# SmartBFT-Go/consensus

Measured on AMD Instinct MI355X. Metric: ECDSA P-256 verifies/sec at batch=1M, higher is better.
Workload: dtype u32

## Files before the change

### consensus_amd/csrc/ed25519_group_kernels.hip

```cpp
#include <hip/hip_runtime.h>

#include <cstdlib>

#include "ed25519_group.h"
#include "ed25519_keyed.h"
#include "ed25519_kernels.h"
#include "group_kernels_common.h"
#include "p256_kernels.h"

namespace sbv {

#ifndef SBV_ED_QPHASE_WAVES
#define SBV_ED_QPHASE_WAVES 3
#endif
#ifndef SBV_ED_GROUP_WAVES
#define SBV_ED_GROUP_WAVES 2
#endif

#ifndef SBV_ED_CHAIN_PRIO
#define SBV_ED_CHAIN_PRIO 0
#endif
static __device__ __forceinline__ void ed_chain_prio() {
#if SBV_ED_CHAIN_PRIO > 0
    __builtin_amdgcn_s_setprio(SBV_ED_CHAIN_PRIO);
#endif
}

__global__ __launch_bounds__(256) void k_ed_group_insert(const uint8_t* __restrict__ tuples, size_t n, GroupState g) {
    const size_t i = (size_t)blockIdx.x * 256 + threadIdx.x;
    (void)i;
    group_insert_block<128, 64, 8>(tuples, n, g);
}

__global__ __launch_bounds__(256) void k_ed_group_split(size_t n, GroupState g) {
    const size_t i = (size_t)blockIdx.x * 256 + threadIdx.x;
    const bool active = i < n;
    u32 s = SBV_GROUP_NONE;
    if (active) s = g.slot_of[g.rep[i]];
    group_split_emit(i, s, active && s == SBV_GROUP_NONE, active && s != SBV_GROUP_NONE, false, g);
}

__global__ __launch_bounds__(64) void k_ed_keytab_bases(const uint8_t* __restrict__ tuples, GroupState g, u32* __restrict__ jbases,
                                                        uint8_t* __restrict__ valid, const u32* __restrict__ tslot, const uint8_t* __restrict__ cold,
                                                        int j_first, int j_last) {
    const u32 lane = blockIdx.x * 64 + threadIdx.x;
    const u32 k = lane >> 2;
    if (k >= group_count(g) || !cold[k]) return;
    edchain_quad_dev q;
    q.r = (int)(lane & 3u);
    edchain_run(q, tuples, k, g, jbases, valid + tslot[k], j_first, j_last);
}

__global__ __launch_bounds__(64) void k_ed_keytab_window(GroupState g, const u32* __restrict__ jbases, u32* __restrict__ tmp,
                                                         aniels* __restrict__ ktab, const u32* __restrict__ tslot, const uint8_t* __restrict__ cold,
                                                         int j_first, int j_count, int parts) {
    const u32 lane = blockIdx.x * 64 + threadIdx.x;
    const u32 part = lane % (u32)parts;
    const u32 kw = lane / (u32)parts;
    const u32 key = kw / (u32)j_count, j = (u32)j_first + kw % (u32)j_count;
    if (key >= group_count(g) || !cold[key]) return;
    const size_t w = (size_t)key * SBV_ED_KEY_WINDOWS + j;
    ed_keytab_window_lane(jbases + w * SBV_ED_JBASE_DWORDS, (int)part, parts,
                          tmp + w * (size_t)(SBV_ED_KEY_PER_WINDOW * SBV_ED_WINDOW_TMP_WORDS) + (size_t)part * (SBV_ED_KEY_PER_WINDOW / parts) * SBV_ED_WINDOW_TMP_WORDS,
// ... 125 lines not shown
                                                                  uint8_t* __restrict__ acc, int j0, int j1, int last) {
    const u32 L = blockIdx.x * SBV_VERIFY_BLOCK + threadIdx.x;
    if (L >= g.counters[1]) return;
    const u32 t = g.grp_idx[L];
    const u32 grp = g.slots[t];
    const bool v = ed_qphase_lane(tuples, t, grp < group_count(g) ? tslot[grp] : SBV_GROUP_NONE, table_slots, ktab, kvalid, gacc, cap, okb, j0, j1, last != 0);
    if (last) acc[t] = v ? SBV_ED_PENDING : 0;
}

__global__ __launch_bounds__(256) void k_ed_finish(const uint8_t* __restrict__ tuples, size_t n, u32* __restrict__ gacc, size_t cap,
                                                   uint8_t* __restrict__ acc, int tuple_major) {
    const size_t i0 = ((size_t)blockIdx.x * 256 + threadIdx.x) * SBV_ED_FINISH_T;
    if (i0 < n) ed_finish_lane(tuples, n, i0, gacc, cap, acc, tuple_major != 0);
}

hipError_t launch_ed25519_verify_grouped(const uint8_t* d_tuples, size_t n, const GroupBuffers& b, const EdGroupBuffers& eb,
                                         u32* d_qtab, const aniels* d_btab, const edcomb& bcomb, uint8_t* d_bitmap, hipStream_t stream,
                                         const GroupSync& y, hipEvent_t* prof, int* prof_pairs) {
    if (n == 0) return hipSuccess;
    GroupState g;
    g.ht = b.ht; g.ht_mask = b.ht_mask; g.rep = b.rep; g.cnt = b.cnt; g.slot_of = b.slot_of; g.group_rep = b.group_rep;
    g.counters = b.counters; g.grp_idx = b.grp_idx; g.ung_idx = b.ung_idx; g.slots = b.slots;
    g.max_groups = b.max_groups; g.seed = b.seed;
    g.gcount = b.gcount; g.gcursor = b.gcount ? b.gcount + b.max_groups : nullptr; g.grp_of = b.grp_of; g.ung_cand = b.ung_cand;
    const size_t sort_lds = (size_t)b.max_groups * sizeof(u32);
    g.sorted = ed25519_group_step_sorted(y, b) ? 1u : 0u;
    group_set_threshold(g, b.min_count);
    const int chunks = y.chunks < 1 ? 1 : (y.chunks > SBV_GROUP_MAX_CHUNKS ? SBV_GROUP_MAX_CHUNKS : y.chunks);
    const int parts = SBV_KEYTAB_PARTS_DEFAULT;
    hipError_t e;
#define SBV_TRY(x) do { if ((e = (x)) != hipSuccess) return e; } while (0)
    SBV_TRY(hipStreamWaitEvent(y.side_a, y.ev_fork, 0));
    SBV_TRY(hipStreamWaitEvent(y.side_a, y.ev_promoted, 0));
    SBV_TRY(hipMemsetAsync(b.ht, 0, ((size_t)b.ht_mask + 1) * sizeof(u32), y.side_a));
    SBV_TRY(hipMemsetAsync(b.cnt, 0, n * sizeof(u32), y.side_a));
    SBV_TRY(hipMemsetAsync(b.counters, 0, SBV_GROUP_COUNTERS * sizeof(u32), y.side_a));
    if (g.sorted) SBV_TRY(hipMemsetAsync(b.gcount, 0, (size_t)b.max_groups * sizeof(u32), y.side_a));
    SBV_TRY(hipMemsetAsync(b.acc, 0, n, y.side_a));
    const unsigned gn = (unsigned)((n + 255) / 256);
    const unsigned gv = (unsigned)((n + SBV_VERIFY_BLOCK - 1) / SBV_VERIFY_BLOCK);
    hipLaunchKernelGGL(k_ed_group_insert, dim3(gn), dim3(256), 0, y.side_a, d_tuples, n, g);
    hipLaunchKernelGGL((k_group_assign_t<128, 64, 8>), dim3(gn), dim3(256), 0, y.side_a, d_tuples, n, g, eb.kc);
    SBV_TRY(hipEventRecord(y.ev_assign, y.side_a));
    hipLaunchKernelGGL((k_key_cache_lookup_t<128, 64, 8>), dim3((b.max_groups + 63) / 64), dim3(64), 0, y.side_a, d_tuples, g, eb.kc, b.tslot, b.cold);
    hipLaunchKernelGGL((k_key_cache_insert_t<128, 64, 8>), dim3((b.max_groups + 63) / 64), dim3(64), 0, y.side_a, d_tuples, g, eb.kc, b.tslot);
    const u32 table_slots = eb.kc.cap + b.max_groups;
    const bool hot_on = eb.wtab && eb.kwide && eb.wide && eb.kc.enabled && g.sorted;
    const HotKeys hk = {eb.wtab, hot_on ? eb.kwide : nullptr, eb.khits, eb.hot, eb.plist, eb.kc.cap, eb.wide_cap, eb.promote_min, eb.wowner, eb.elist};
    const uint8_t* wide = hot_on ? eb.wide : nullptr;
    if (hot_on) SBV_TRY(hipEventRecord(y.ev_cache, y.side_a));
    SBV_TRY(hipStreamWaitEvent(y.side_b, y.ev_assign, 0));
    if (hot_on) SBV_TRY(hipMemsetAsync(eb.hot + 1, 0, 3 * sizeof(u32), y.side_b));
    if (g.sorted) {
        const unsigned tiles = (unsigned)((n + SBV_SORT_TILE - 1) / SBV_SORT_TILE);
        hipLaunchKernelGGL(k_group_classify, dim3(gn), dim3(256), 0, y.side_b, n, g, b.ung_cand, b.counters + 4);
        hipLaunchKernelGGL(k_group_sort_count, dim3(tiles), dim3(1024), sort_lds, y.side_b, n, g);
        hipLaunchKernelGGL(k_group_sort_scan, dim3(1), dim3(1024), 0, y.side_b, g);
        hipLaunchKernelGGL(k_group_sort_scatter, dim3(tiles), dim3(1024), sort_lds, y.side_b, n, g);
    } else {
        hipLaunchKernelGGL(k_ed_group_split, dim3(gn), dim3(256), 0, y.side_b, n, g);
    }
    if (hot_on) {
        SBV_TRY(hipStreamWaitEvent(y.side_b, y.ev_cache, 0));
        hipLaunchKernelGGL(k_ed_hot_class, dim3(64), dim3(256), 0, y.side_b, g, b.tslot, b.cold, hk, eb.wide);
    }
    SBV_TRY(hipEventRecord(y.ev_split, y.side_b));
    hipLaunchKernelGGL(k_ed_gphase, dim3(gv), dim3(SBV_VERIFY_BLOCK), 0, stream, d_tuples, n, bcomb, b.gacc, b.gacc_cap, eb.okb, (int)g.sorted);
    if (hot_on) SBV_TRY(hipEventRecord(y.ev_class, stream));
    SBV_TRY(hipStreamWaitEvent(stream, y.ev_split, 0));
    for (int c = 0; c < chunks; ++c) {
        const int j_first = SBV_ED_KEY_WINDOWS * c / chunks, j_end = SBV_ED_KEY_WINDOWS * (c + 1) / chunks;
        hipLaunchKernelGGL(k_ed_keytab_bases, dim3((b.max_groups * 4u + 63) / 64), dim3(64), 0, y.side_a, d_tuples, g, b.jbases, eb.kvalid,
                           b.tslot, b.cold, j_first, j_end - 1);
        SBV_TRY(hipEventRecord(y.ev_bases[c], y.side_a));
    }
    SBV_TRY(hipStreamWaitEvent(y.side_a, y.ev_split, 0));
    static const bool quad_env = [] { const char* e = getenv("SBV_ED_UNGROUPED_QUAD"); return e && atoi(e) != 0; }();
    static const bool keep_keys = [] { const char* e = getenv("SBV_ED_UNGROUPED_KEYS"); return !e || atoi(e) != 0; }();
// ... 130 lines not shown
```

### consensus_amd/csrc/group_kernels_common.h

```cpp
#pragma once
#include <hip/hip_runtime.h>

#include "p256_group.h"

namespace sbv {

__device__ __forceinline__ u32 group_count(const GroupState& g) {
    const u32 c = g.counters[0];
    return c < g.max_groups ? c : g.max_groups;
}

template <int STRIDE, int OFF, int WORDS>
static __device__ __forceinline__ void group_insert_block(const uint8_t* __restrict__ tuples, size_t n, const GroupState& g) {
    __shared__ u32 skey[512], scnt[512];
    const unsigned tid = threadIdx.x;
    for (unsigned t = tid; t < 512; t += blockDim.x) { skey[t] = 0xFFFFFFFFu; scnt[t] = 0; }
    __syncthreads();
    const size_t i = (size_t)blockIdx.x * blockDim.x + tid;
    u32 mine = 0xFFFFFFFFu;
    bool want = false;
    if (i < n) {
        mine = group_find_rep_t<STRIDE, OFF, WORDS>(tuples, i, g);
        want = group_sampled((u32)i, g.sample_mask);
    }
    unsigned long long todo = __ballot(want);
    const int lane = (int)(tid & 63u);
    if (todo) {
        const int first = __ffsll((long long)todo) - 1;
        const u32 r0 = (u32)__shfl((int)mine, first, 64);
        if (__popcll(__ballot(want && mine == r0)) < 2) {
            if (want) atomicAdd(&g.cnt[mine], 1u);
            todo = 0;
        }
    }
    while (todo) {
        const int leader = __ffsll((long long)todo) - 1;
        const u32 r = (u32)__shfl((int)mine, leader, 64);
        const unsigned long long same = __ballot(want && mine == r);
        if (lane == leader) {
            const u32 c = (u32)__popcll(same);
            u32 h = (r * 0x9E3779B1u) >> 23;
            for (int probes = 0; probes < 512; ++probes) {
                const u32 prev = atomicCAS(&skey[h], 0xFFFFFFFFu, r);
                if (prev == 0xFFFFFFFFu || prev == r) { atomicAdd(&scnt[h], c); break; }
                h = (h + 1u) & 511u;
            }
        }
        todo &= ~same;
    }
    __syncthreads();
    for (unsigned t = tid; t < 512; t += blockDim.x)
        if (skey[t] != 0xFFFFFFFFu) atomicAdd(&g.cnt[skey[t]], scnt[t]);
}

template <int STRIDE, int OFF, int WORDS>
static __global__ __launch_bounds__(256) void k_group_assign_t(const uint8_t* __restrict__ tuples, size_t n, GroupState g, KeyCache kc) {
    const size_t i = (size_t)blockIdx.x * 256 + threadIdx.x;
    if (i < n) group_assign_lane_t<STRIDE, OFF, WORDS>(tuples, i, g, kc);
}
static __global__ __launch_bounds__(256) void k_group_assign(const uint8_t* __restrict__ tuples, size_t n, GroupState g, KeyCache kc) {
    const size_t i = (size_t)blockIdx.x * 256 + threadIdx.x;
    if (i < n) group_assign_lane(tuples, i, g, kc);
}

template <int STRIDE, int OFF, int WORDS>
static __global__ __launch_bounds__(64) void k_key_cache_lookup_t(const uint8_t* __restrict__ tuples, GroupState g, KeyCache kc,
                                                                  u32* __restrict__ tslot, uint8_t* __restrict__ cold) {
    const u32 k = blockIdx.x * 64 + threadIdx.x;
    if (k == 0) { kc.count[1] = 0; kc.count[2] = 0; }
    if (k >= group_count(g)) return;
    key_cache_phase_lookup<STRIDE, OFF, WORDS>(tuples, g, kc, k, tslot, cold);
}
template <int STRIDE, int OFF, int WORDS>
static __global__ __launch_bounds__(64) void k_key_cache_insert_t(const uint8_t* __restrict__ tuples, GroupState g, KeyCache kc,
                                                                  u32* __restrict__ tslot) {
    const u32 k = blockIdx.x * 64 + threadIdx.x;
    if (k >= group_count(g)) return;
    key_cache_phase_insert<STRIDE, OFF, WORDS>(tuples, g, kc, k, tslot);
}

struct HotKeys { const void* wtab; u32* kwide; u32* khits; u32* hot; u32* plist; u32 cache_cap, wide_cap, promote_min; u32* wowner; u32* elist; };
static __device__ __forceinline__ u32 promote_live(const u32* hot) { const u32 c = hot[1]; return c < SBV_PROMOTE_MAX ? c : SBV_PROMOTE_MAX; }
static __global__ __launch_bounds__(256) void k_hot_decay(HotKeys hk) {
    const u32 slot = blockIdx.x * 256 + threadIdx.x;
    if (slot < hk.cache_cap) hot_decay_lane(slot, hk.khits);
}
static __global__ __launch_bounds__(256) void k_promote_select(GroupState g, const u32* __restrict__ tslot, const uint8_t* __restrict__ kvalid, HotKeys hk) {
    const u32 groups = group_count(g);
    for (u32 k = blockIdx.x * 256 + threadIdx.x; k < groups; k += gridDim.x * 256)
        group_promote_select_lane(k, tslot, kvalid, hk.cache_cap, hk.kwide, hk.khits, hk.promote_min, hk.wide_cap, hk.hot, hk.plist, hk.elist);
}
#define SBV_HOT_POOL_MAX 4096u
static __global__ __launch_bounds__(1024) void k_promote_evict(HotKeys hk) {
    __shared__ u32 taken[SBV_HOT_POOL_MAX / 32];
    __shared__ u32 sh_h[16], sh_w[16];
    __shared__ u32 entries;
    const u32 tid = threadIdx.x;
    const u32 ncand = hk.hot[3] < SBV_PROMOTE_MAX ? hk.hot[3] : SBV_PROMOTE_MAX;
    if (ncand == 0 || hk.wide_cap > SBV_HOT_POOL_MAX) return;
    for (u32 i = tid; i < SBV_HOT_POOL_MAX / 32; i += 1024) taken[i] = 0;
    if (tid == 0) entries = hk.hot[1] < SBV_PROMOTE_MAX ? hk.hot[1] : SBV_PROMOTE_MAX;
    __syncthreads();
    {
        u32 mc = 0;
        for (u32 c = tid; c < ncand; c += 1024) { const u32 h = hk.khits[hk.elist[c]]; mc = h > mc ? h : mc; }
        u32 bh, bw;
        hot_evict_scan(hk.khits, hk.wowner, taken, hk.wide_cap, hk.cache_cap, tid, 1024u, bh, bw);
        for (int off = 32; off >= 1; off >>= 1) {
            const u32 om = (u32)__shfl_xor((int)mc, off, 64), oh = (u32)__shfl_xor((int)bh, off, 64);
            mc = om > mc ? om : mc;
            bh = oh < bh ? oh : bh;
// ... 193 lines not shown
```

### consensus_amd/csrc/k256_group_kernels.hip

```cpp
#include <hip/hip_runtime.h>

#include <thread>
#include <vector>

#include "group_kernels_common.h"
#include "k256_group.h"
#include "k256_keyed.h"
#include "p256_kernels.h"

namespace sbv {

struct KGlobalTupleG {
    const u32* p;
    __device__ __forceinline__ u32 operator[](int i) const { return p[i]; }
};
#define SBV_K256_PREP_T 8
__global__ __launch_bounds__(64) void k_k256_prep_chunk(const uint8_t* __restrict__ tuples, size_t n, Scratch s, int T) {
    const size_t first = (size_t)blockIdx.x * 64 * (size_t)T + threadIdx.x;
    auto words = [&](size_t idx) { return KGlobalTupleG{reinterpret_cast<const u32*>(tuples + idx * 160)}; };
    k256_prep_chunk(words, n, s, first, (size_t)64, T);
}
__global__ __launch_bounds__(256) void k_k256_group_insert(const uint8_t* __restrict__ tuples, size_t n, GroupState g) {
    group_insert_block<160, 96, 16>(tuples, n, g);
}
// ... 123 lines not shown
}
__global__ __launch_bounds__(64) void k_k256_promote_build(const u32* __restrict__ plist, const u32* __restrict__ hot, const kapt* __restrict__ ktab, u32 cache_cap,
                                                           u32* __restrict__ tmp, kapt* __restrict__ wtab, u32 wide_cap) {
    const u32 total = promote_live(hot) * SBV_K256_WIDE_LANES;
    const u32 gid = blockIdx.x * 64 + threadIdx.x;
    u32* mine = tmp + (size_t)gid * SBV_K256_WIDE_TMP_WORDS;
    for (u32 item = gid; item < total; item += gridDim.x * 64) {
        const u32 i = item / SBV_K256_WIDE_LANES, lane = item % SBV_K256_WIDE_LANES;
        const u32 slot = plist[2 * i], w = plist[2 * i + 1];
        if (slot >= cache_cap || w >= wide_cap) continue;
        k256_widetab_lane(ktab + (size_t)slot * SBV_K256_KEYTAB_ENTRIES, lane, mine, wtab + (size_t)w * SBV_K256_WIDE_ENTRIES);
    }
}

hipError_t launch_k256_verify_grouped(const uint8_t* d_tuples, const Scratch& s_in, size_t n, const GroupBuffers& b, const KeyPool& kp, u32* d_qtab,
                                      const kapt* d_gtab, const kapt* d_gcomb, int gcomb_bits, uint8_t* d_bitmap, hipStream_t stream, const GroupSync& y, hipEvent_t* prof, int* prof_pairs) {
    if (n == 0) return hipSuccess;
    GroupState g;
    g.ht = b.ht; g.ht_mask = b.ht_mask; g.rep = b.rep; g.cnt = b.cnt; g.slot_of = b.slot_of; g.group_rep = b.group_rep;
    g.counters = b.counters; g.grp_idx = b.grp_idx; g.ung_idx = b.ung_idx; g.slots = b.slots; g.max_groups = b.max_groups; g.seed = b.seed;
    g.gcount = b.gcount; g.gcursor = b.gcount + b.max_groups; g.grp_of = b.grp_of; g.ung_cand = b.ung_cand;
    g.sorted = k256_group_step_sorted(y, b) ? 1u : 0u;
    group_set_threshold(g, b.min_count);
    Scratch s = s_in;
    s.rec = b.rec;
    const size_t sort_lds = (size_t)b.max_groups * sizeof(u32);
    kapt* ktab = reinterpret_cast<kapt*>(kp.ktab);
    uint8_t* kvalid = kp.kvalid;
    const u32 table_slots = kp.kc.cap + b.max_groups;
    hipError_t e;
#define SBV_TRY(x) do { if ((e = (x)) != hipSuccess) return e; } while (0)
    SBV_TRY(hipStreamWaitEvent(y.side_a, y.ev_fork, 0));
    SBV_TRY(hipStreamWaitEvent(y.side_a, y.ev_promoted, 0));
    SBV_TRY(hipMemsetAsync(b.ht, 0, ((size_t)b.ht_mask + 1) * sizeof(u32), y.side_a));
    SBV_TRY(hipMemsetAsync(b.cnt, 0, n * sizeof(u32), y.side_a));
    SBV_TRY(hipMemsetAsync(b.counters, 0, SBV_GROUP_COUNTERS * sizeof(u32), y.side_a));
    SBV_TRY(hipMemsetAsync(b.gcount, 0, (size_t)b.max_groups * sizeof(u32), y.side_a));
    const unsigned gn = (unsigned)((n + 255) / 256);
    const unsigned gv = (unsigned)((n + SBV_VERIFY_BLOCK - 1) / SBV_VERIFY_BLOCK);
    hipLaunchKernelGGL(k_k256_group_insert, dim3(gn), dim3(256), 0, y.side_a, d_tuples, n, g);
    hipLaunchKernelGGL(k_group_assign, dim3(gn), dim3(256), 0, y.side_a, d_tuples, n, g, kp.kc);
    SBV_TRY(hipEventRecord(y.ev_assign, y.side_a));
    hipLaunchKernelGGL((k_key_cache_lookup_t<160, 96, 16>), dim3((b.max_groups + 63) / 64), dim3(64), 0, y.side_a, d_tuples, g, kp.kc, b.tslot, b.cold);
    hipLaunchKernelGGL((k_key_cache_insert_t<160, 96, 16>), dim3((b.max_groups + 63) / 64), dim3(64), 0, y.side_a, d_tuples, g, kp.kc, b.tslot);
    const bool hot_on = kp.wtab && kp.kwide && kp.wide && kp.build_blocks && kp.kc.enabled && g.sorted;
    const HotKeys hk = {kp.wtab, hot_on ? kp.kwide : nullptr, kp.khits, kp.hot, kp.plist, kp.kc.cap, kp.wide_cap, kp.promote_min, kp.wowner, kp.elist};
    const uint8_t* wide = hot_on ? kp.wide : nullptr;
    if (hot_on) SBV_TRY(hipEventRecord(y.ev_cache, y.side_a));
    {
        const size_t per_block = (size_t)64 * SBV_K256_PREP_T;
        hipLaunchKernelGGL(k_k256_prep_chunk, dim3((unsigned)((n + per_block - 1) / per_block)), dim3(64), 0, stream, d_tuples, n, s, SBV_K256_PREP_T);
    }
    SBV_TRY(hipStreamWaitEvent(y.side_b, y.ev_assign, 0));
    if (hot_on) SBV_TRY(hipMemsetAsync(kp.hot + 1, 0, 3 * sizeof(u32), y.side_b));
    hipLaunchKernelGGL(k_group_classify, dim3(gn), dim3(256), 0, y.side_b, n, g, b.ung_cand, b.counters + 4);
    hipLaunchKernelGGL(k_k256_keycheck, dim3(gn), dim3(256), 0, y.side_b, d_tuples, g, b.acc);
    const unsigned tiles = (unsigned)((n + SBV_SORT_TILE - 1) / SBV_SORT_TILE);
    hipLaunchKernelGGL(k_group_sort_count, dim3(tiles), dim3(1024), sort_lds, y.side_b, n, g);
    hipLaunchKernelGGL(k_group_sort_scan, dim3(1), dim3(1024), 0, y.side_b, g);
    hipLaunchKernelGGL(k_group_sort_scatter, dim3(tiles), dim3(1024), sort_lds, y.side_b, n, g);
    if (hot_on) {
        SBV_TRY(hipStreamWaitEvent(y.side_b, y.ev_cache, 0));
        hipLaunchKernelGGL(k_k256_hot_class, dim3(64), dim3(256), 0, y.side_b, g, b.tslot, b.cold, hk, kp.wide);
    }
    SBV_TRY(hipEventRecord(y.ev_split, y.side_b));
    SBV_TRY(hipStreamWaitEvent(stream, y.ev_split, 0));
    hipLaunchKernelGGL(k_k256_gphase_generic, dim3(2 * gv), dim3(SBV_VERIFY_BLOCK), 0, stream, s, g, d_qtab, d_gtab, kgcomb_make(d_gcomb, gcomb_bits), b.gacc, b.acc, gv);
    if (hot_on) SBV_TRY(hipEventRecord(y.ev_class, stream));
    const int chunks = 2;
    for (int c = 0; c < chunks; ++c) {
        const int j_first = SBV_GTAB_WINDOWS * c / chunks, j_end = SBV_GTAB_WINDOWS * (c + 1) / chunks, j_count = j_end - j_first;
        hipLaunchKernelGGL(k_k256_chain, dim3((b.max_groups * 4 + 63) / 64), dim3(64), 0, y.side_a, d_tuples, g, b.jstate, b.bases, kvalid, b.tslot, b.cold, j_first, j_end - 1);
        SBV_TRY(hipEventRecord(y.ev_bases[c], y.side_a));
        hipStream_t tb = y.tstreams > 1 && y.side_t && (c & 1) ? y.side_t : y.side_b;
        SBV_TRY(hipStreamWaitEvent(tb, y.ev_bases[c], 0));
        const size_t wl = (size_t)b.max_groups * j_count * 2, fl = (size_t)b.max_groups * j_count * 7;
        hipLaunchKernelGGL(k_k256_rows, dim3((unsigned)((wl + 63) / 64)), dim3(64), 0, tb, g, b.bases, b.tmp, ktab, b.tslot, b.cold, j_first, j_count);
// ... 41 lines not shown
```

### consensus_amd/csrc/p256_group.h

```cpp
#pragma once
#include "p256_core.h"
#include "p256_comb29.h"

namespace sbv {

#if defined(__HIP_DEVICE_COMPILE__)
#define SBV_ATOMIC_CAS(p, cmp, val) atomicCAS((p), (cmp), (val))
#define SBV_ATOMIC_ADD(p, v) atomicAdd((p), (v))
#else
SBV_HD u32 host_cas(u32* p, u32 cmp, u32 val) { const u32 old = *p; if (old == cmp) *p = val; return old; }
SBV_HD u32 host_add(u32* p, u32 v) { const u32 old = *p; *p = old + v; return old; }
#define SBV_ATOMIC_CAS(p, cmp, val) host_cas((p), (cmp), (val))
#define SBV_ATOMIC_ADD(p, v) host_add((p), (v))
#endif

#define SBV_GROUP_NONE 0xFFFFFFFFu
#define SBV_GROUP_COUNTERS 12
#define SBV_GROUP_MAX_PROBES 64u

struct GroupState {
    u32* ht;
    u32 ht_mask;
    u32* rep;
    u32* cnt;
// ... 30 lines not shown
    h ^= h >> 15;
    h *= 0x85EBCA77u;
    return ((h >> 24) & sample_mask) == 0;
}

SBV_HD const u32* tuple_key_words(const uint8_t* tuples, size_t i) {
    return reinterpret_cast<const u32*>(tuples + i * 160 + 96);
}

SBV_HD bool key29_load(const uint8_t* tuples, size_t idx, fe29& x, fe29& y) {
    const u32* k = tuple_key_words(tuples, idx);
    u256 qx, qy;
    SBV_UNROLL
    for (int l = 0; l < 8; ++l) { qx.v[l] = bswap32(k[7 - l]); qy.v[l] = bswap32(k[8 + 7 - l]); }
    const fe p_ = fe_p();
    f29_from_plain(x, qx);
    f29_from_plain(y, qy);
    fe29 lhs, t, rhs;
    f29_sqr(lhs, y);
    f29_sqr(t, x);
    f29_mul(rhs, t, x);
    f29_sub(rhs, rhs, x);
    f29_sub(rhs, rhs, x);
    f29_sub(rhs, rhs, x);
    f29_add(rhs, rhs, f29_b());
    f29_sub(t, lhs, rhs);
    return lt256(qx, p_) && lt256(qy, p_) && f29_is_zero(t);
}
SBV_HD bool tuple_key_ok(const uint8_t* tuples, size_t idx) {
    fe29 x, y;
    return key29_load(tuples, idx, x, y);
}

template <int STRIDE, int OFF, int WORDS>
SBV_HD u32 group_find_rep_t(const uint8_t* tuples, size_t i, const GroupState& g) {
    const u32* k = reinterpret_cast<const u32*>(tuples + i * STRIDE + OFF);
    u32 w[WORDS];
    SBV_UNROLL
    for (int j = 0; j < WORDS; ++j) w[j] = k[j];
    u32 h = 0x9E3779B1u ^ g.seed;
    SBV_UNROLL
    for (int j = 0; j < WORDS; ++j) {
        h = (h ^ w[j]) * 0x85EBCA77u;
        h ^= h >> 15;
    }
    h = (h ^ (g.seed * 0x27D4EB2Fu)) * 0xC2B2AE3Du;
    h ^= h >> 16;
    u32 slot = h & g.ht_mask;
    u32 mine = (u32)i;
    for (u32 probes = 0; probes < SBV_GROUP_MAX_PROBES && probes <= g.ht_mask; ++probes) {
        u32 v = g.ht[slot];
        if (v == 0) v = SBV_ATOMIC_CAS(&g.ht[slot], 0u, (u32)i + 1u);
        if (v == 0) break;
        const u32* o = reinterpret_cast<const u32*>(tuples + (size_t)(v - 1) * STRIDE + OFF);
        u32 diff = 0;
        SBV_UNROLL
        for (int j = 0; j < WORDS; ++j) diff |= o[j] ^ w[j];
        if (diff == 0) { mine = v - 1; break; }
        slot = (slot + 1) & g.ht_mask;
    }
    g.rep[i] = mine;
    return mine;
}
template <int STRIDE, int OFF, int WORDS>
SBV_HD void group_insert_lane_t(const uint8_t* tuples, size_t i, const GroupState& g) {
    const u32 mine = group_find_rep_t<STRIDE, OFF, WORDS>(tuples, i, g);
    if (group_sampled((u32)i, g.sample_mask)) SBV_ATOMIC_ADD(&g.cnt[mine], 1u);
}
SBV_HD void group_insert_lane(const uint8_t* tuples, size_t i, const GroupState& g) { group_insert_lane_t<160, 96, 16>(tuples, i, g); }

SBV_HD bool group_split_lane(const uint8_t* tuples, size_t i, const GroupState& g, uint8_t* acc) {
    const u32 s = g.slot_of[g.rep[i]];
    if (s == SBV_GROUP_NONE) {
        g.slots[i] = SBV_GROUP_NONE;
        if (!tuple_key_ok(tuples, i)) {
            acc[i] = 0;
            SBV_ATOMIC_ADD(&g.counters[3], 1u);
            return false;
        }
        g.ung_idx[SBV_ATOMIC_ADD(&g.counters[2], 1u)] = (u32)i;
    } else {
        g.slots[i] = s;
        if (!g.sorted) g.grp_idx[SBV_ATOMIC_ADD(&g.counters[1], 1u)] = (u32)i;
    }
    return true;
}

// ... 43 lines not shown
struct KeyCache {
    u32* ht;
    u32 ht_mask;
    u32* keys;
    u32* count;
    u32 cap;
    u32 enabled;
    u32 seed;
};
SBV_HD u32 key_hash16(const u32 w[16], u32 seed) {
    u32 h = 0x9E3779B1u ^ seed;
    SBV_UNROLL
    for (int j = 0; j < 16; ++j) {
        h = (h ^ w[j]) * 0x85EBCA77u;
        h ^= h >> 15;
    }
    h = (h ^ (seed * 0x27D4EB2Fu)) * 0xC2B2AE3Du;
    return h ^ (h >> 16);
}
SBV_HD u32 key_cache_lookup(const KeyCache& kc, const u32 w[16]) {
    u32 p = key_hash16(w, kc.seed) & kc.ht_mask;
    for (u32 probes = 0; probes < SBV_GROUP_MAX_PROBES && probes <= kc.ht_mask; ++probes) {
        const u32 v = kc.ht[p];
        if (v == 0) return SBV_GROUP_NONE;
        const u32* o = kc.keys + (size_t)(v - 1) * 16;
        u32 diff = 0;
        SBV_UNROLL
        for (int j = 0; j < 16; ++j) diff |= o[j] ^ w[j];
        if (diff == 0) return v - 1;
        p = (p + 1) & kc.ht_mask;
    }
    return SBV_GROUP_NONE;
}
SBV_HD u32 key_cache_insert(const KeyCache& kc, const u32 w[16]) {
    if (kc.count[0] >= kc.cap) return SBV_GROUP_NONE;
    const u32 slot = SBV_ATOMIC_ADD(&kc.count[0], 1u);
    if (slot >= kc.cap) return SBV_GROUP_NONE;
    u32* o = kc.keys + (size_t)slot * 16;
    SBV_UNROLL
    for (int j = 0; j < 16; ++j) o[j] = w[j];
    u32 p = key_hash16(w, kc.seed) & kc.ht_mask;
    for (u32 probes = 0; probes < SBV_GROUP_MAX_PROBES && probes <= kc.ht_mask; ++probes) {
        if (SBV_ATOMIC_CAS(&kc.ht[p], 0u, slot + 1u) == 0u) break;
        p = (p + 1) & kc.ht_mask;
    }
    return slot;
}
template <int STRIDE, int OFF, int WORDS>
SBV_HD void key_words16_t(const uint8_t* tuples, size_t i, u32 w[16]) {
    const u32* k = reinterpret_cast<const u32*>(tuples + i * STRIDE + OFF);
    SBV_UNROLL
    for (int j = 0; j < 16; ++j) w[j] = j < WORDS ? k[j] : 0u;
}
template <int STRIDE, int OFF, int WORDS>
SBV_HD void group_assign_lane_t(const uint8_t* tuples, size_t i, const GroupState& g, const KeyCache& kc) {
    u32 s = SBV_GROUP_NONE;
    if (g.rep[i] == (u32)i) {
        bool take = g.cnt[i] >= g.min_samples;
        if (!take && kc.enabled) {
            u32 w[16];
            key_words16_t<STRIDE, OFF, WORDS>(tuples, i, w);
            take = key_cache_lookup(kc, w) != SBV_GROUP_NONE;
        }
        if (take) {
            const u32 got = SBV_ATOMIC_ADD(&g.counters[0], 1u);
            if (got < g.max_groups) { s = got; g.group_rep[got] = (u32)i; }
        }
    }
    g.slot_of[i] = s;
}
SBV_HD void group_assign_lane(const uint8_t* tuples, size_t i, const GroupState& g, const KeyCache& kc) {
    group_assign_lane_t<160, 96, 16>(tuples, i, g, kc);
}
SBV_HD void group_assign_lane(size_t i, const GroupState& g) {
    KeyCache off = {};
    group_assign_lane(nullptr, i, g, off);
}

template <int STRIDE, int OFF, int WORDS>
// ... 124 lines not shown
```

### consensus_amd/csrc/p256_group_kernels.hip

```cpp
#include <hip/hip_runtime.h>

#include <cstdlib>

#include "group_kernels_common.h"
#include "p256_kernels.h"
#include "p256_keytab29.h"

#ifndef SBV_GPHASE_WAVES
#define SBV_GPHASE_WAVES 3
#endif
#ifndef SBV_COMB29_WAVES
#define SBV_COMB29_WAVES 2
#endif
#ifndef SBV_QPHASE_WAVES
#define SBV_QPHASE_WAVES 3
#endif

namespace sbv {

__global__ __launch_bounds__(256) void k_group_insert(const uint8_t* __restrict__ tuples, size_t n, GroupState g) {
    group_insert_block<160, 96, 16>(tuples, n, g);
}
__global__ __launch_bounds__(256) void k_group_split(const uint8_t* __restrict__ tuples, size_t n, GroupState g, uint8_t* __restrict__ acc) {
    const size_t i = (size_t)blockIdx.x * 256 + threadIdx.x;
// ... 423 lines not shown
        u256 r;
        rec_load256(r, s.rec, t, SBV_REC_R);
        acc[t] = ok && pt29_rx_matches(R, r) ? 1 : 0;
    }
}

hipError_t launch_p256_verify_grouped(const uint8_t* d_tuples, const Scratch& s_in, size_t n, const GroupBuffers& b,
                                      u32* d_qtab, const apt* d_g16, const gcomb& d_g16r, uint8_t* d_bitmap, hipStream_t stream,
                                      const GroupSync& y, hipEvent_t after_prep, hipEvent_t* prof, int* prof_pairs) {
    if (n == 0) return hipSuccess;
    GroupState g;
    g.ht = b.ht; g.ht_mask = b.ht_mask; g.rep = b.rep; g.cnt = b.cnt; g.slot_of = b.slot_of; g.group_rep = b.group_rep;
    g.counters = b.counters; g.grp_idx = b.grp_idx; g.ung_idx = b.ung_idx; g.slots = b.slots;
    g.max_groups = b.max_groups; g.seed = b.seed;
    g.gcount = b.gcount; g.gcursor = b.gcount ? b.gcount + b.max_groups : nullptr; g.grp_of = b.grp_of; g.ung_cand = b.ung_cand;
    const size_t sort_lds = (size_t)(b.max_groups > SBV_SORT_LDS_GROUPS ? SBV_SORT_LDS_GROUPS : b.max_groups) * sizeof(u32);
    g.sorted = p256_group_step_sorted(y, s_in, b) ? 1u : 0u;
    Scratch s = s_in;
    if (!g.sorted) s.rec = nullptr;
    if (b.sample_shift >= 0) group_set_sampling(g, b.min_count, (u32)b.sample_shift);
    else group_set_threshold(g, b.min_count);
    const int chunks = y.chunks < 1 ? 1 : (y.chunks > SBV_GROUP_MAX_CHUNKS ? SBV_GROUP_MAX_CHUNKS : y.chunks);
    const bool coop = g.sorted && y.coop_max && n <= y.coop_max;
    const u32 full_min = coop ? 0u : b.full_min;
    const u32 table_slots = b.kc.cap + b.max_groups;
    const bool hot_on = b.wtab && b.kwide && b.kc.enabled && g.sorted;
    const HotKeys hk = {b.wtab, hot_on ? b.kwide : nullptr, b.khits, b.hot, b.plist, b.kc.cap, b.wide_cap, b.promote_min, b.wowner, b.elist};
    const widekeys wk = hot_on ? widekeys_make(b.wtab, b.kwide, SBV_HOT_BITS) : widekeys_none();
    static const bool q_lds = [] { const char* v = getenv("SBV_QPHASE_LDS"); return v && v[0] == '1'; }();
    hipError_t e;
#define SBV_TRY(x) do { if ((e = (x)) != hipSuccess) return e; } while (0)
    SBV_TRY(hipStreamWaitEvent(y.side_a, y.ev_fork, 0));
    SBV_TRY(hipStreamWaitEvent(y.side_a, y.ev_promoted, 0));
    SBV_TRY(hipMemsetAsync(b.ht, 0, ((size_t)b.ht_mask + 1) * sizeof(u32), y.side_a));
    SBV_TRY(hipMemsetAsync(b.cnt, 0, n * sizeof(u32), y.side_a));
    SBV_TRY(hipMemsetAsync(b.counters, 0, SBV_GROUP_COUNTERS * sizeof(u32), y.side_a));
    if (g.sorted) SBV_TRY(hipMemsetAsync(b.gcount, 0, (size_t)b.max_groups * sizeof(u32), y.side_a));
    const unsigned gn = (unsigned)((n + 255) / 256);
    const unsigned gv = (unsigned)((n + SBV_VERIFY_BLOCK - 1) / SBV_VERIFY_BLOCK);
    hipLaunchKernelGGL(k_group_insert, dim3(gn), dim3(256), 0, y.side_a, d_tuples, n, g);
    hipLaunchKernelGGL(k_group_assign, dim3(gn), dim3(256), 0, y.side_a, d_tuples, n, g, b.kc);
    SBV_TRY(hipEventRecord(y.ev_assign, y.side_a));
    hipLaunchKernelGGL((k_key_cache_lookup_t<160, 96, 16>), dim3((b.max_groups + 63) / 64), dim3(64), 0, y.side_a, d_tuples, g, b.kc, b.tslot, b.cold);
    hipLaunchKernelGGL((k_key_cache_insert_t<160, 96, 16>), dim3((b.max_groups + 63) / 64), dim3(64), 0, y.side_a, d_tuples, g, b.kc, b.tslot);
    SBV_TRY(hipEventRecord(y.ev_cache, y.side_a));
    const size_t pbt = prep_block_tuples(n);
    const unsigned pblocks = (unsigned)((n + pbt - 1) / pbt);
    SBV_TRY(launch_p256_prep_blocks(d_tuples, n, s, stream, 0, pblocks));
    SBV_TRY(hipStreamWaitEvent(y.side_b, y.ev_assign, 0));
    if (hot_on) SBV_TRY(hipMemsetAsync(b.hot + 1, 0, 3 * sizeof(u32), y.side_b));
    if (!g.sorted) hipLaunchKernelGGL(k_group_split, dim3(gn), dim3(256), 0, y.side_b, d_tuples, n, g, b.acc);
    if (g.sorted) {
        hipLaunchKernelGGL(k_group_classify, dim3(gn), dim3(256), 0, y.side_b, n, g, b.ung_cand, b.counters + 4);
        hipLaunchKernelGGL(k_group_keycheck, dim3(gn), dim3(256), 0, y.side_b, d_tuples, g, b.acc);
        const unsigned tiles = (unsigned)((n + SBV_SORT_TILE - 1) / SBV_SORT_TILE);
        hipLaunchKernelGGL(k_group_sort_count, dim3(tiles), dim3(1024), sort_lds, y.side_b, n, g);
        hipLaunchKernelGGL(k_group_sort_scan, dim3(1), dim3(1024), 0, y.side_b, g);
    }
    if (g.sorted) {
        const unsigned tiles = (unsigned)((n + SBV_SORT_TILE - 1) / SBV_SORT_TILE);
        hipLaunchKernelGGL(k_group_sort_scatter, dim3(tiles), dim3(1024), sort_lds, y.side_b, n, g);
    }
    SBV_TRY(hipEventRecord(y.ev_split, y.side_b));
    SBV_TRY(hipStreamWaitEvent(y.side_b, y.ev_cache, 0));
    hipLaunchKernelGGL(k_group_table_class, dim3(64), dim3(256), 0, y.side_b, g, b.tslot, b.cold, b.kfull, table_slots, full_min, b.full, b.needfill, hk, b.wide);
    SBV_TRY(hipEventRecord(y.ev_class, y.side_b));
    SBV_TRY(hipStreamWaitEvent(stream, y.ev_assign, 0));
    SBV_TRY(hipStreamWaitEvent(stream, y.ev_split, 0));
    if (after_prep) SBV_TRY(hipEventRecord(after_prep, stream));
    if (coop) {
        hipLaunchKernelGGL(k_gphase_generic, dim3(gv), dim3(SBV_VERIFY_BLOCK), 0, stream, d_tuples, s, n, g, d_qtab, d_g16, d_g16r, b.gacc, b.acc, gv, (size_t)0, n);
    } else if (g.sorted && y.gsplit_min && n >= y.gsplit_min) {
        hipLaunchKernelGGL(k_gphase_generic, dim3(gv), dim3(SBV_VERIFY_BLOCK), 0, stream, d_tuples, s, n, g, d_qtab, d_g16, d_g16r, b.gacc, b.acc, gv, (size_t)0, n);
        hipLaunchKernelGGL(k_gphase_sorted, dim3(gv), dim3(SBV_VERIFY_BLOCK), 0, stream, s, g, d_g16r, b.gacc);
    } else {
        hipLaunchKernelGGL(k_gphase_generic, dim3(gv + gv), dim3(SBV_VERIFY_BLOCK), 0, stream, d_tuples, s, n, g, d_qtab, d_g16, d_g16r, b.gacc, b.acc, gv, (size_t)0, n);
    }
// ... 88 lines not shown
```

Baseline: 327.4 million.

## Fuse group-state memsets into one clear kernel and skip disabled key-cache passes

Replaces four or five separate hipMemsetAsync calls with one k_group_clear kernel that zeroes every array using 16-byte stores. When the key cache is disabled, the lookup and insert kernels are skipped, and the assign kernel writes tslot and cold directly. The cache insert is rewritten to reserve slots per wavefront with a single atomic, and key loads use uint4 vector reads. This cuts launch count and atomic contention on the side stream. The risk is that the vector loads assume 16-byte-aligned keys and the clear kernel needs more care than a plain memset.

```diff
diff --git a/consensus_amd/csrc/ed25519_group_kernels.hip b/consensus_amd/csrc/ed25519_group_kernels.hip
--- a/consensus_amd/csrc/ed25519_group_kernels.hip
+++ b/consensus_amd/csrc/ed25519_group_kernels.hip
@@ -27,8 +27,6 @@
 }
 
 __global__ __launch_bounds__(256) void k_ed_group_insert(const uint8_t* __restrict__ tuples, size_t n, GroupState g) {
-    const size_t i = (size_t)blockIdx.x * 256 + threadIdx.x;
-    (void)i;
     group_insert_block<128, 64, 8>(tuples, n, g);
 }
 
@@ -220,18 +218,26 @@
 #define SBV_TRY(x) do { if ((e = (x)) != hipSuccess) return e; } while (0)
     SBV_TRY(hipStreamWaitEvent(y.side_a, y.ev_fork, 0));
     SBV_TRY(hipStreamWaitEvent(y.side_a, y.ev_promoted, 0));
-    SBV_TRY(hipMemsetAsync(b.ht, 0, ((size_t)b.ht_mask + 1) * sizeof(u32), y.side_a));
-    SBV_TRY(hipMemsetAsync(b.cnt, 0, n * sizeof(u32), y.side_a));
-    SBV_TRY(hipMemsetAsync(b.counters, 0, SBV_GROUP_COUNTERS * sizeof(u32), y.side_a));
-    if (g.sorted) SBV_TRY(hipMemsetAsync(b.gcount, 0, (size_t)b.max_groups * sizeof(u32), y.side_a));
-    SBV_TRY(hipMemsetAsync(b.acc, 0, n, y.side_a));
+    {
+        GroupClear gc = {};
+        gc.p[0] = b.ht; gc.words[0] = (size_t)b.ht_mask + 1;
+        gc.p[1] = b.cnt; gc.words[1] = n;
+        gc.p[2] = b.counters; gc.words[2] = SBV_GROUP_COUNTERS;
+        if (g.sorted) { gc.p[3] = b.gcount; gc.words[3] = b.max_groups; }
+        gc.p[4] = reinterpret_cast<u32*>(b.acc); gc.words[4] = n / 4;
+        gc.tail = b.acc + (n & ~(size_t)3); gc.tail_bytes = (u32)(n & 3);
+        if (!eb.kc.enabled) gc.kc_count = eb.kc.count;
+        SBV_TRY(launch_group_clear(gc, y.side_a));
+    }
     const unsigned gn = (unsigned)((n + 255) / 256);
     const unsigned gv = (unsigned)((n + SBV_VERIFY_BLOCK - 1) / SBV_VERIFY_BLOCK);
     hipLaunchKernelGGL(k_ed_group_insert, dim3(gn), dim3(256), 0, y.side_a, d_tuples, n, g);
-    hipLaunchKernelGGL((k_group_assign_t<128, 64, 8>), dim3(gn), dim3(256), 0, y.side_a, d_tuples, n, g, eb.kc);
+    hipLaunchKernelGGL((k_group_assign_t<128, 64, 8>), dim3(gn), dim3(256), 0, y.side_a, d_tuples, n, g, eb.kc, b.tslot, b.cold);
     SBV_TRY(hipEventRecord(y.ev_assign, y.side_a));
-    hipLaunchKernelGGL((k_key_cache_lookup_t<128, 64, 8>), dim3((b.max_groups + 63) / 64), dim3(64), 0, y.side_a, d_tuples, g, eb.kc, b.tslot, b.cold);
-    hipLaunchKernelGGL((k_key_cache_insert_t<128, 64, 8>), dim3((b.max_groups + 63) / 64), dim3(64), 0, y.side_a, d_tuples, g, eb.kc, b.tslot);
+    if (eb.kc.enabled) {
+        hipLaunchKernelGGL((k_key_cache_lookup_t<128, 64, 8>), dim3((b.max_groups + 63) / 64), dim3(64), 0, y.side_a, d_tuples, g, eb.kc, b.tslot, b.cold);
+        hipLaunchKernelGGL((k_key_cache_insert_t<128, 64, 8>), dim3((b.max_groups + 63) / 64), dim3(64), 0, y.side_a, d_tuples, g, eb.kc, b.tslot);
+    }
     const u32 table_slots = eb.kc.cap + b.max_groups;
     const bool hot_on = eb.wtab && eb.kwide && eb.wide && eb.kc.enabled && g.sorted;
     const HotKeys hk = {eb.wtab, hot_on ? eb.kwide : nullptr, eb.khits, eb.hot, eb.plist, eb.kc.cap, eb.wide_cap, eb.promote_min, eb.wowner, eb.elist};
diff --git a/consensus_amd/csrc/group_kernels_common.h b/consensus_amd/csrc/group_kernels_common.h
--- a/consensus_amd/csrc/group_kernels_common.h
+++ b/consensus_amd/csrc/group_kernels_common.h
@@ -53,14 +53,57 @@
         if (skey[t] != 0xFFFFFFFFu) atomicAdd(&g.cnt[skey[t]], scnt[t]);
 }
 
-template <int STRIDE, int OFF, int WORDS>
-static __global__ __launch_bounds__(256) void k_group_assign_t(const uint8_t* __restrict__ tuples, size_t n, GroupState g, KeyCache kc) {
+#define SBV_GROUP_CLEAR_ARRAYS 5
+struct GroupClear { u32* p[SBV_GROUP_CLEAR_ARRAYS]; size_t words[SBV_GROUP_CLEAR_ARRAYS]; uint8_t* tail; u32 tail_bytes; u32* kc_count; };
+static __global__ __launch_bounds__(256) void k_group_clear(GroupClear c) {
+    const size_t t = (size_t)blockIdx.x * 256 + threadIdx.x, T = (size_t)gridDim.x * 256;
+#pragma unroll
+    for (int a = 0; a < SBV_GROUP_CLEAR_ARRAYS; ++a) {
+        u32* p = c.p[a];
+        const size_t w = c.words[a];
+        if (!p || !w) continue;
+        size_t head = ((16u - (unsigned)(reinterpret_cast<uintptr_t>(p) & 15u)) & 15u) / 4u;
+        if (head > w) head = w;
+        const size_t quads = (w - head) / 4;
+        uint4* q = reinterpret_cast<uint4*>(p + head);
+        for (size_t i = t; i < quads; i += T) q[i] = make_uint4(0u, 0u, 0u, 0u);
+        const size_t done = head + 4 * quads;
+        if (t < head) p[t] = 0;
+        if (t < w - done) p[done + t] = 0;
+    }
+    if (t == 0) {
+        for (u32 k = 0; k < c.tail_bytes; ++k) c.tail[k] = 0;
+        if (c.kc_count) { c.kc_count[1] = 0; c.kc_count[2] = 0; }
+    }
+}
+static inline hipError_t launch_group_clear(const GroupClear& c, hipStream_t stream) {
+    size_t quads = 0;
+    for (int a = 0; a < SBV_GROUP_CLEAR_ARRAYS; ++a) if (c.p[a]) quads += c.words[a] / 4;
+    size_t blocks = (quads + 255) / 256;
+    blocks = blocks < 1 ? 1 : (blocks > 1024 ? 1024 : blocks);
+    hipLaunchKernelGGL(k_group_clear, dim3((unsigned)blocks), dim3(256), 0, stream, c);
+    return hipGetLastError();
+}
+
+template <int STRIDE, int OFF, int WORDS>
+static __device__ __forceinline__ void group_assign_block(const uint8_t* __restrict__ tuples, size_t n, const GroupState& g, const KeyCache& kc,
+                                                          u32* __restrict__ tslot, uint8_t* __restrict__ cold) {
     const size_t i = (size_t)blockIdx.x * 256 + threadIdx.x;
-    if (i < n) group_assign_lane_t<STRIDE, OFF, WORDS>(tuples, i, g, kc);
-}
-static __global__ __launch_bounds__(256) void k_group_assign(const uint8_t* __restrict__ tuples, size_t n, GroupState g, KeyCache kc) {
-    const size_t i = (size_t)blockIdx.x * 256 + threadIdx.x;
-    if (i < n) group_assign_lane(tuples, i, g, kc);
+    if (i >= n) return;
+    group_assign_lane_t<STRIDE, OFF, WORDS>(tuples, i, g, kc);
+    if (!kc.enabled) {
+        const u32 k = g.slot_of[i];
+        if (k != SBV_GROUP_NONE) { tslot[k] = kc.cap + k; cold[k] = 1; }
+    }
+}
+template <int STRIDE, int OFF, int WORDS>
+static __global__ __launch_bounds__(256) void k_group_assign_t(const uint8_t* __restrict__ tuples, size_t n, GroupState g, KeyCache kc,
+                                                              u32* __restrict__ tslot, uint8_t* __restrict__ cold) {
+    group_assign_block<STRIDE, OFF, WORDS>(tuples, n, g, kc, tslot, cold);
+}
+static __global__ __launch_bounds__(256) void k_group_assign(const uint8_t* __restrict__ tuples, size_t n, GroupState g, KeyCache kc,
+                                                             u32* __restrict__ tslot, uint8_t* __restrict__ cold) {
+    group_assign_block<160, 96, 16>(tuples, n, g, kc, tslot, cold);
 }
 
 template <int STRIDE, int OFF, int WORDS>
@@ -75,8 +118,35 @@
 static __global__ __launch_bounds__(64) void k_key_cache_insert_t(const uint8_t* __restrict__ tuples, GroupState g, KeyCache kc,
                                                                   u32* __restrict__ tslot) {
     const u32 k = blockIdx.x * 64 + threadIdx.x;
-    if (k >= group_count(g)) return;
-    key_cache_phase_insert<STRIDE, OFF, WORDS>(tuples, g, kc, k, tslot);
+    const bool active = k < group_count(g);
+    const bool miss = active && tslot[k] == SBV_GROUP_NONE;
+    const unsigned long long mm = __ballot(miss), mh = __ballot(active && !miss);
+    if (!kc.enabled) {
+        if (miss) tslot[k] = kc.cap + k;
+        return;
+    }
+    const int lane = (int)(threadIdx.x & 63u);
+    if (lane == 0) {
+        if (mh) atomicAdd(&kc.count[1], (u32)__popcll(mh));
+        if (mm) atomicAdd(&kc.count[2], (u32)__popcll(mm));
+    }
+    if (!mm) return;
+    const int leader = __ffsll((long long)mm) - 1;
+    u32 base = SBV_GROUP_NONE;
+    if (lane == leader && kc.count[0] < kc.cap) base = atomicAdd(&kc.count[0], (u32)__popcll(mm));
+    base = (u32)__shfl((int)base, leader, 64);
+    if (!miss) return;
+    u32 slot = SBV_GROUP_NONE;
+    if (base != SBV_GROUP_NONE) {
+        const u32 s = base + (u32)__popcll(mm & ((1ull << lane) - 1ull));
+        if (s >= base && s < kc.cap) {
+            u32 w[16];
+            key_cache_group_key_t<STRIDE, OFF, WORDS>(tuples, g, k, w);
+            key_cache_publish(kc, w, s);
+            slot = s;
+        }
+    }
+    tslot[k] = slot == SBV_GROUP_NONE ? kc.cap + k : slot;
 }
 
 struct HotKeys { const void* wtab; u32* kwide; u32* khits; u32* hot; u32* plist; u32 cache_cap, wide_cap, promote_min; u32* wowner; u32* elist; };
diff --git a/consensus_amd/csrc/k256_group_kernels.hip b/consensus_amd/csrc/k256_group_kernels.hip
--- a/consensus_amd/csrc/k256_group_kernels.hip
+++ b/consensus_amd/csrc/k256_group_kernels.hip
@@ -179,17 +179,24 @@
 #define SBV_TRY(x) do { if ((e = (x)) != hipSuccess) return e; } while (0)
     SBV_TRY(hipStreamWaitEvent(y.side_a, y.ev_fork, 0));
     SBV_TRY(hipStreamWaitEvent(y.side_a, y.ev_promoted, 0));
-    SBV_TRY(hipMemsetAsync(b.ht, 0, ((size_t)b.ht_mask + 1) * sizeof(u32), y.side_a));
-    SBV_TRY(hipMemsetAsync(b.cnt, 0, n * sizeof(u32), y.side_a));
-    SBV_TRY(hipMemsetAsync(b.counters, 0, SBV_GROUP_COUNTERS * sizeof(u32), y.side_a));
-    SBV_TRY(hipMemsetAsync(b.gcount, 0, (size_t)b.max_groups * sizeof(u32), y.side_a));
+    {
+        GroupClear gc = {};
+        gc.p[0] = b.ht; gc.words[0] = (size_t)b.ht_mask + 1;
+        gc.p[1] = b.cnt; gc.words[1] = n;
+        gc.p[2] = b.counters; gc.words[2] = SBV_GROUP_COUNTERS;
+        gc.p[3] = b.gcount; gc.words[3] = b.max_groups;
+        if (!kp.kc.enabled) gc.kc_count = kp.kc.count;
+        SBV_TRY(launch_group_clear(gc, y.side_a));
+    }
     const unsigned gn = (unsigned)((n + 255) / 256);
     const unsigned gv = (unsigned)((n + SBV_VERIFY_BLOCK - 1) / SBV_VERIFY_BLOCK);
     hipLaunchKernelGGL(k_k256_group_insert, dim3(gn), dim3(256), 0, y.side_a, d_tuples, n, g);
-    hipLaunchKernelGGL(k_group_assign, dim3(gn), dim3(256), 0, y.side_a, d_tuples, n, g, kp.kc);
+    hipLaunchKernelGGL(k_group_assign, dim3(gn), dim3(256), 0, y.side_a, d_tuples, n, g, kp.kc, b.tslot, b.cold);
     SBV_TRY(hipEventRecord(y.ev_assign, y.side_a));
-    hipLaunchKernelGGL((k_key_cache_lookup_t<160, 96, 16>), dim3((b.max_groups + 63) / 64), dim3(64), 0, y.side_a, d_tuples, g, kp.kc, b.tslot, b.cold);
-    hipLaunchKernelGGL((k_key_cache_insert_t<160, 96, 16>), dim3((b.max_groups + 63) / 64), dim3(64), 0, y.side_a, d_tuples, g, kp.kc, b.tslot);
+    if (kp.kc.enabled) {
+        hipLaunchKernelGGL((k_key_cache_lookup_t<160, 96, 16>), dim3((b.max_groups + 63) / 64), dim3(64), 0, y.side_a, d_tuples, g, kp.kc, b.tslot, b.cold);
+        hipLaunchKernelGGL((k_key_cache_insert_t<160, 96, 16>), dim3((b.max_groups + 63) / 64), dim3(64), 0, y.side_a, d_tuples, g, kp.kc, b.tslot);
+    }
     const bool hot_on = kp.wtab && kp.kwide && kp.wide && kp.build_blocks && kp.kc.enabled && g.sorted;
     const HotKeys hk = {kp.wtab, hot_on ? kp.kwide : nullptr, kp.khits, kp.hot, kp.plist, kp.kc.cap, kp.wide_cap, kp.promote_min, kp.wowner, kp.elist};
     const uint8_t* wide = hot_on ? kp.wide : nullptr;
diff --git a/consensus_amd/csrc/p256_group.h b/consensus_amd/csrc/p256_group.h
--- a/consensus_amd/csrc/p256_group.h
+++ b/consensus_amd/csrc/p256_group.h
@@ -86,12 +86,26 @@
     return key29_load(tuples, idx, x, y);
 }
 
+template <int WORDS>
+SBV_HD void key_words_load_t(const uint8_t* key, u32 w[WORDS]) {
+#if defined(__HIP_DEVICE_COMPILE__)
+    static_assert(WORDS % 4 == 0, "whole 16-byte pieces");
+    const uint4* q = reinterpret_cast<const uint4*>(key);
+    SBV_UNROLL
+    for (int j = 0; j < WORDS / 4; ++j) {
+        const uint4 v = q[j];
+        w[4 * j] = v.x; w[4 * j + 1] = v.y; w[4 * j + 2] = v.z; w[4 * j + 3] = v.w;
+    }
+#else
+    const u32* k = reinterpret_cast<const u32*>(key);
+    SBV_UNROLL
+    for (int j = 0; j < WORDS; ++j) w[j] = k[j];
+#endif
+}
 template <int STRIDE, int OFF, int WORDS>
 SBV_HD u32 group_find_rep_t(const uint8_t* tuples, size_t i, const GroupState& g) {
-    const u32* k = reinterpret_cast<const u32*>(tuples + i * STRIDE + OFF);
     u32 w[WORDS];
-    SBV_UNROLL
-    for (int j = 0; j < WORDS; ++j) w[j] = k[j];
+    key_words_load_t<WORDS>(tuples + i * STRIDE + OFF, w);
     u32 h = 0x9E3779B1u ^ g.seed;
     SBV_UNROLL
     for (int j = 0; j < WORDS; ++j) {
@@ -106,7 +120,8 @@
         u32 v = g.ht[slot];
         if (v == 0) v = SBV_ATOMIC_CAS(&g.ht[slot], 0u, (u32)i + 1u);
         if (v == 0) break;
-        const u32* o = reinterpret_cast<const u32*>(tuples + (size_t)(v - 1) * STRIDE + OFF);
+        u32 o[WORDS];
+        key_words_load_t<WORDS>(tuples + (size_t)(v - 1) * STRIDE + OFF, o);
         u32 diff = 0;
         SBV_UNROLL
         for (int j = 0; j < WORDS; ++j) diff |= o[j] ^ w[j];
@@ -216,10 +231,15 @@
     }
     return SBV_GROUP_NONE;
 }
+SBV_HD void key_cache_publish(const KeyCache& kc, const u32 w[16], u32 slot);
 SBV_HD u32 key_cache_insert(const KeyCache& kc, const u32 w[16]) {
     if (kc.count[0] >= kc.cap) return SBV_GROUP_NONE;
     const u32 slot = SBV_ATOMIC_ADD(&kc.count[0], 1u);
     if (slot >= kc.cap) return SBV_GROUP_NONE;
+    key_cache_publish(kc, w, slot);
+    return slot;
+}
+SBV_HD void key_cache_publish(const KeyCache& kc, const u32 w[16], u32 slot) {
     u32* o = kc.keys + (size_t)slot * 16;
     SBV_UNROLL
     for (int j = 0; j < 16; ++j) o[j] = w[j];
@@ -228,7 +248,6 @@
         if (SBV_ATOMIC_CAS(&kc.ht[p], 0u, slot + 1u) == 0u) break;
         p = (p + 1) & kc.ht_mask;
     }
-    return slot;
 }
 template <int STRIDE, int OFF, int WORDS>
 SBV_HD void key_words16_t(const uint8_t* tuples, size_t i, u32 w[16]) {
diff --git a/consensus_amd/csrc/p256_group_kernels.hip b/consensus_amd/csrc/p256_group_kernels.hip
--- a/consensus_amd/csrc/p256_group_kernels.hip
+++ b/consensus_amd/csrc/p256_group_kernels.hip
@@ -479,17 +479,24 @@
 #define SBV_TRY(x) do { if ((e = (x)) != hipSuccess) return e; } while (0)
     SBV_TRY(hipStreamWaitEvent(y.side_a, y.ev_fork, 0));
     SBV_TRY(hipStreamWaitEvent(y.side_a, y.ev_promoted, 0));
-    SBV_TRY(hipMemsetAsync(b.ht, 0, ((size_t)b.ht_mask + 1) * sizeof(u32), y.side_a));
-    SBV_TRY(hipMemsetAsync(b.cnt, 0, n * sizeof(u32), y.side_a));
-    SBV_TRY(hipMemsetAsync(b.counters, 0, SBV_GROUP_COUNTERS * sizeof(u32), y.side_a));
-    if (g.sorted) SBV_TRY(hipMemsetAsync(b.gcount, 0, (size_t)b.max_groups * sizeof(u32), y.side_a));
+    {
+        GroupClear gc = {};
+        gc.p[0] = b.ht; gc.words[0] = (size_t)b.ht_mask + 1;
+        gc.p[1] = b.cnt; gc.words[1] = n;
+        gc.p[2] = b.counters; gc.words[2] = SBV_GROUP_COUNTERS;
+        if (g.sorted) { gc.p[3] = b.gcount; gc.words[3] = b.max_groups; }
+        if (!b.kc.enabled) gc.kc_count = b.kc.count;
+        SBV_TRY(launch_group_clear(gc, y.side_a));
+    }
     const unsigned gn = (unsigned)((n + 255) / 256);
     const unsigned gv = (unsigned)((n + SBV_VERIFY_BLOCK - 1) / SBV_VERIFY_BLOCK);
     hipLaunchKernelGGL(k_group_insert, dim3(gn), dim3(256), 0, y.side_a, d_tuples, n, g);
-    hipLaunchKernelGGL(k_group_assign, dim3(gn), dim3(256), 0, y.side_a, d_tuples, n, g, b.kc);
+    hipLaunchKernelGGL(k_group_assign, dim3(gn), dim3(256), 0, y.side_a, d_tuples, n, g, b.kc, b.tslot, b.cold);
     SBV_TRY(hipEventRecord(y.ev_assign, y.side_a));
-    hipLaunchKernelGGL((k_key_cache_lookup_t<160, 96, 16>), dim3((b.max_groups + 63) / 64), dim3(64), 0, y.side_a, d_tuples, g, b.kc, b.tslot, b.cold);
-    hipLaunchKernelGGL((k_key_cache_insert_t<160, 96, 16>), dim3((b.max_groups + 63) / 64), dim3(64), 0, y.side_a, d_tuples, g, b.kc, b.tslot);
+    if (b.kc.enabled) {
+        hipLaunchKernelGGL((k_key_cache_lookup_t<160, 96, 16>), dim3((b.max_groups + 63) / 64), dim3(64), 0, y.side_a, d_tuples, g, b.kc, b.tslot, b.cold);
+        hipLaunchKernelGGL((k_key_cache_insert_t<160, 96, 16>), dim3((b.max_groups + 63) / 64), dim3(64), 0, y.side_a, d_tuples, g, b.kc, b.tslot);
+    }
     SBV_TRY(hipEventRecord(y.ev_cache, y.side_a));
     const size_t pbt = prep_block_tuples(n);
     const unsigned pblocks = (unsigned)((n + pbt - 1) / pbt);
```

Measured after the change: 332.9 million (median of 6 runs). 1.02x the previous value.
